# HiLab-git/WSL4MIS

Measured on AMD Instinct MI355X. Metric: training slices/sec (256x256, bs64, unet_cct pCE+GatedCRF), higher is better.
Workload: dtype f32; 1 GPU; unet_cct pce_gatedcrf r=5, 256x256x1 4-class synthetic scribble slices, batch 64/GPU, SGD+poly LR; global_batch=64, parallelism=dp1, crf_radius=5, conv_precision=f32

## Files before the change

### wsl4mis_amd/csrc/wsl_bn.hip

```cpp
#include <stdlib.h>

#include "wsl_rt.h"

namespace wsl {

constexpr int kChunk = 4096;

constexpr int kFinalizeWideFrom = 2048;
static inline int finalize_threads(int nblk) { return nblk >= kFinalizeWideFrom ? 1024 : kThreads; }
template <int NV>
__device__ __forceinline__ void finalize_merge_waves(double (&v)[NV], double* red) {
  const int nw = blockDim.x >> 6, w = threadIdx.x >> 6;
#pragma unroll
  for (int m = 32; m >= 1; m >>= 1)
#pragma unroll
    for (int k = 0; k < NV; ++k) v[k] += __shfl_xor(v[k], m);
  if ((threadIdx.x & 63) == 0)
#pragma unroll
    for (int k = 0; k < NV; ++k) red[k * 16 + w] = v[k];
  __syncthreads();
#pragma unroll
  for (int k = 0; k < NV; ++k) {
    double t[16];
#pragma unroll
// ... 79 lines not shown
      best = v[0];
#pragma unroll
      for (int k = 1; k < 4; ++k)
        if (v[k] > best) best = v[k];
    } else {
#pragma unroll
      for (int k = 0; k < 4; ++k) {
        const int64_t off = (int64_t)(2 * oy + (k >> 1)) * W + 2 * ox + (k & 1);
        const float v = src_value(s, n, c, n * s.bs + c * HW + off, ((int64_t)n * s.C + c) * HW + off);
        if (k == 0 || v > best) best = v;
      }
    }
    out[((int64_t)n * s.C + c) * Ho * Wo + o] = best;
  }
}

__global__ __launch_bounds__(256) void feat_grad_combine_kernel(WslSrc f, const float* ga, int64_t ga_bs,
                                                                const float* gb, int64_t gb_bs, const float* gb_cmask,
                                                                const float* gp, float* g, int H, int W) {
  const int c = blockIdx.y, n = blockIdx.z;
  const int Hc = (H + 1) / 2, Wc = (W + 1) / 2, Ho = H / 2, Wo = W / 2;
  const int64_t HW = (int64_t)H * W;
  const float cm = gb_cmask ? gb_cmask[(int64_t)n * f.C + c] : 1.f;
  const int base = blockIdx.x * kChunk;
  for (int o = base + threadIdx.x; o < base + kChunk && o < Hc * Wc; o += kThreads) {
    const int cy = o / Wc, cx = o - cy * Wc;
    int arg = -1;
    float gpool = 0.f;
    if (gp && cy < Ho && cx < Wo) {
      float best = 0.f;
#pragma unroll
      for (int k = 0; k < 4; ++k) {
        const int64_t off = (int64_t)(2 * cy + (k >> 1)) * W + 2 * cx + (k & 1);
        const float v = src_value(f, n, c, n * f.bs + c * HW + off, ((int64_t)n * f.C + c) * HW + off);
        if (k == 0 || v > best) best = v, arg = k;
      }
      gpool = gp[((int64_t)n * f.C + c) * Ho * Wo + (int64_t)cy * Wo + cx];
    }
#pragma unroll
    for (int k = 0; k < 4; ++k) {
      const int y = 2 * cy + (k >> 1), x = 2 * cx + (k & 1);
      if (y < H && x < W) {
        const int64_t off = (int64_t)y * W + x;
        float v = 0.f;
        if (ga) v = ga[n * ga_bs + c * HW + off];
        if (gb) v = fmaf(gb[n * gb_bs + c * HW + off], cm, v);
        if (k == arg) v += gpool;
        g[((int64_t)n * f.C + c) * HW + off] = v;
      }
    }
  }
}

__global__ __launch_bounds__(256) void feat_grad_combine_bn_kernel(WslSrc f, const float* ga, int64_t ga_bs, const float* gb,
                                                                   int64_t gb_bs, const float* gb_cmask, const float* gp,
                                                                   float* g, int H, int W, const float* bn_mean,
                                                                   const float* bn_invstd, float* bn_part) {
  __shared__ float red[8];
  const int c = blockIdx.y, n = blockIdx.z;
  const int Hc = (H + 1) / 2, Wc = (W + 1) / 2, Ho = H / 2, Wo = W / 2;
  const int64_t HW = (int64_t)H * W;
  const float cm = gb_cmask ? gb_cmask[(int64_t)n * f.C + c] : 1.f;
  const float sc = f.scale[c], sh = f.shift[c], mean = bn_mean[c], invstd = bn_invstd[c];
  const float* fy = f.x + n * f.bs + c * HW;
  float s1 = 0.f, s2 = 0.f;
  const int base = blockIdx.x * kChunk;
  const bool vec = !(H & 1) && !(W & 1) && !(HW & 1) && !(f.bs & 1) && !(ga_bs & 1) && !(gb_bs & 1) &&
                   !(reinterpret_cast<uintptr_t>(f.x) & 7) && !(reinterpret_cast<uintptr_t>(g) & 7) &&
                   !(reinterpret_cast<uintptr_t>(ga) & 7) && !(reinterpret_cast<uintptr_t>(gb) & 7);
  for (int o = base + threadIdx.x; o < base + kChunk && o < Hc * Wc; o += kThreads) {
    const int cy = o / Wc, cx = o - cy * Wc;
    float yv[4], zv[4];
    bool in[4];
    if (vec) {
      const float2 t = *reinterpret_cast<const float2*>(fy + (int64_t)(2 * cy) * W + 2 * cx);
      const float2 b = *reinterpret_cast<const float2*>(fy + (int64_t)(2 * cy + 1) * W + 2 * cx);
      yv[0] = t.x, yv[1] = t.y, yv[2] = b.x, yv[3] = b.y;
#pragma unroll
      for (int k = 0; k < 4; ++k) in[k] = true, zv[k] = fmaf(yv[k], sc, sh);
    } else {
#pragma unroll
      for (int k = 0; k < 4; ++k) {
        const int y = 2 * cy + (k >> 1), x = 2 * cx + (k & 1);
        in[k] = y < H && x < W;
        yv[k] = in[k] ? fy[(int64_t)y * W + x] : 0.f;
        zv[k] = fmaf(yv[k], sc, sh);
      }
    }
    int arg = -1;
    float gpool = 0.f;
    if (gp && cy < Ho && cx < Wo) {
      float best = 0.f;
#pragma unroll
      for (int k = 0; k < 4; ++k) {
        const float v = leaky(zv[k]);
        if (k == 0 || v > best) best = v, arg = k;
      }
      gpool = gp[((int64_t)n * f.C + c) * Ho * Wo + (int64_t)cy * Wo + cx];
    }
    float av[4] = {0.f, 0.f, 0.f, 0.f}, bv[4] = {0.f, 0.f, 0.f, 0.f};
    if (vec) {
      const int64_t o0 = c * HW + (int64_t)(2 * cy) * W + 2 * cx;
      if (ga) {
        const float2 t = *reinterpret_cast<const float2*>(ga + n * ga_bs + o0), b = *reinterpret_cast<const float2*>(ga + n * ga_bs + o0 + W);
        av[0] = t.x, av[1] = t.y, av[2] = b.x, av[3] = b.y;
      }
      if (gb) {
        const float2 t = *reinterpret_cast<const float2*>(gb + n * gb_bs + o0), b = *reinterpret_cast<const float2*>(gb + n * gb_bs + o0 + W);
        bv[0] = t.x, bv[1] = t.y, bv[2] = b.x, bv[3] = b.y;
      }
    }
    float vout[4];
#pragma unroll
    for (int k = 0; k < 4; ++k) {
      vout[k] = 0.f;
      if (in[k]) {
        const int64_t off = (int64_t)(2 * cy + (k >> 1)) * W + 2 * cx + (k & 1);
        float v = 0.f;
        if (ga) v = vec ? av[k] : ga[n * ga_bs + c * HW + off];
        if (gb) v = fmaf(vec ? bv[k] : gb[n * gb_bs + c * HW + off], cm, v);
        if (k == arg) v += gpool;
        if (!vec) g[((int64_t)n * f.C + c) * HW + off] = v;
        vout[k] = v;
        const float d = zv[k] > 0.f ? v : WSL_LEAKY_SLOPE * v;
        s1 += d;
        s2 = fmaf(d, (yv[k] - mean) * invstd, s2);
      }
    }
    if (vec) {
      float* go = g + ((int64_t)n * f.C + c) * HW + (int64_t)(2 * cy) * W + 2 * cx;
      *reinterpret_cast<float2*>(go) = make_float2(vout[0], vout[1]);
      *reinterpret_cast<float2*>(go + W) = make_float2(vout[2], vout[3]);
    }
  }
  s1 = block_sum(s1, red);
  s2 = block_sum(s2, red + 4);
  if (threadIdx.x == 0) {
    float* dst = bn_part + (((int64_t)n * gridDim.x + blockIdx.x) * f.C + c) * 2;
    dst[0] = s1;
    dst[1] = s2;
  }
}

struct BnBwdP {
  const float* g;
  int64_t g_bs;
  const float* y;
  const float* mean;
  const float* invstd;
  const float* gamma;
  const float* beta;
  const uint8_t* emask;
  float es;
  int C, HW, chunks;
  int g_is_d = 0;
};

__device__ __forceinline__ float bn_dz(const BnBwdP& p, int n, int c, int i, float sc, float sh, float mean, float invstd,
                                       float* xhat) {
  const int64_t idx = ((int64_t)n * p.C + c) * p.HW + i;
  const float yv = p.y[idx];
  float d = p.g[n * p.g_bs + (int64_t)c * p.HW + i];
  *xhat = (yv - mean) * invstd;
  if (p.g_is_d) return d;
  if (p.emask) d = p.emask[idx] ? d * p.es : 0.f;
  const float z = fmaf(yv, sc, sh);
  return z > 0.f ? d : WSL_LEAKY_SLOPE * d;
}

__global__ __launch_bounds__(256) void bnact_bwd_reduce_kernel(BnBwdP p, float* part) {
  __shared__ float red[8];
  const int c = blockIdx.y, n = blockIdx.z;
  const float mean = p.mean[c], invstd = p.invstd[c];
  const float sc = p.gamma[c] * invstd, sh = fmaf(-mean, sc, p.beta[c]);
  float s1 = 0.f, s2 = 0.f;
  const int base = blockIdx.x * kChunk;
  for (int i = base + threadIdx.x; i < base + kChunk && i < p.HW; i += kThreads) {
    float xh;
    const float d = bn_dz(p, n, c, i, sc, sh, mean, invstd, &xh);
    s1 += d;
    s2 = fmaf(d, xh, s2);
  }
  s1 = block_sum(s1, red);
  s2 = block_sum(s2, red + 4);
  if (threadIdx.x == 0) {
// ... 512 lines not shown
    return WSL_EWORKSPACE;
  }
  BnBwdP p{g, g_bs, y, mean, invstd, gamma, beta, emask, emask_scale, C, H * W, cdiv(H * W, kChunk)};
  p.g_is_d = g_is_d;
  ProfScope ps(PF_BN_BWD, 0.0, (double)N * C * H * W * (12.0 + (emask && !g_is_d ? 1.0 : 0.0)), stream);
  float* coef = static_cast<float*>(ws);
  dim3 grid(p.chunks, C, N);
  auto al16 = [](const void* q) { return (reinterpret_cast<uintptr_t>(q) & 15) == 0; };
  const bool vec = (H * W) % 4 == 0 && (g_bs % 4) == 0 && al16(g) && al16(y) && al16(dy) &&
                   (!emask || (reinterpret_cast<uintptr_t>(emask) & 3) == 0);
  bnact_bwd_finalize_launch(part, nblk, C, channel_major, (double)N * H * W, dgamma, dbeta, coef, stream);
  uint32_t* pmax = dy_amax ? reinterpret_cast<uint32_t*>(coef + 2 * (size_t)C) : nullptr;
  if (vec) WSL_LAUNCH(bnact_bwd_apply4_kernel, grid, dim3(kThreads), 0, stream, p, coef, dy, pmax);
  else WSL_LAUNCH(bnact_bwd_apply_kernel, grid, dim3(kThreads), 0, stream, p, coef, dy, pmax);
  if (dy_amax) WSL_LAUNCH(amax_fold_kernel, dim3(WSL_SP_AMAX_SLOTS), dim3(kThreads), 0, stream, pmax, N * p.chunks * C, dy_amax);
  return check_launch("bnact_bwd_finish");
}

extern "C" int wsl_bnact_bwd_finish_amax(const float* g, int64_t g_bs, const float* y, const float* mean, const float* invstd,
                                         const float* gamma, const float* beta, const uint8_t* emask, float emask_scale, float* dy,
                                         float* dgamma, float* dbeta, int N, int C, int H, int W, const float* part, int nblk,
                                         int channel_major, void* ws, size_t ws_bytes, uint32_t* dy_amax, void* stream) {
  return bnact_bwd_finish_impl(g, g_bs, y, mean, invstd, gamma, beta, emask, emask_scale, dy, dgamma, dbeta, N, C, H, W, part, nblk,
                               channel_major, ws, ws_bytes, dy_amax, 0, stream);
}

extern "C" int wsl_bnact_bwd_finish_d_amax(const float* d, int64_t d_bs, const float* y, const float* mean, const float* invstd,
                                           const float* gamma, const float* beta, float* dy, float* dgamma, float* dbeta, int N, int C,
                                           int H, int W, const float* part, int nblk, int channel_major, void* ws, size_t ws_bytes,
                                           uint32_t* dy_amax, void* stream) {
  return bnact_bwd_finish_impl(d, d_bs, y, mean, invstd, gamma, beta, nullptr, 1.f, dy, dgamma, dbeta, N, C, H, W, part, nblk,
                               channel_major, ws, ws_bytes, dy_amax, 1, stream);
}

extern "C" int wsl_bnact_bwd_finish(const float* g, int64_t g_bs, const float* y, const float* mean, const float* invstd,
                                    const float* gamma, const float* beta, const uint8_t* emask, float emask_scale, float* dy,
                                    float* dgamma, float* dbeta, int N, int C, int H, int W, const float* part, int nblk,
                                    int channel_major, void* ws, size_t ws_bytes, void* stream) {
  return wsl_bnact_bwd_finish_amax(g, g_bs, y, mean, invstd, gamma, beta, emask, emask_scale, dy, dgamma, dbeta, N, C, H, W, part,
                                   nblk, channel_major, ws, ws_bytes, nullptr, stream);
}

extern "C" int wsl_feat_grad_combine_blocks(int N, int H, int W) {
  return N > 0 && H > 0 && W > 0 ? N * cdiv(((H + 1) / 2) * ((W + 1) / 2), kChunk) : 0;
}

extern "C" int wsl_feat_grad_combine_bn(const WslSrc* f, const float* ga, int64_t ga_bs, const float* gb, int64_t gb_bs,
                                        const float* gb_cmask, const float* gp, float* g, int N, int H, int W,
                                        const float* bn_mean, const float* bn_invstd, float* bn_part, void* stream) {
  WSL_REQUIRE(f && f->x && f->scale && f->shift && !f->emask && !f->cmask && g && N > 0 && H > 0 && W > 0 && f->C > 0,
              "feat_grad_combine_bn: the feature must be a plain BatchNorm + LeakyReLU source");
  WSL_REQUIRE(bn_mean && bn_invstd && bn_part, "feat_grad_combine_bn: null BatchNorm argument");
  ProfScope ps(PF_POOL_FANIN, 0.0, (double)N * f->C * H * W * (4.0 * (ga ? 1 : 0) + 4.0 * (gb ? 1 : 0) + (gp ? 1.0 : 0.0) + 8.0), stream);
  WSL_LAUNCH(feat_grad_combine_bn_kernel, dim3(cdiv(((H + 1) / 2) * ((W + 1) / 2), kChunk), f->C, N), dim3(kThreads), 0,
             stream, *f, ga, ga_bs, gb, gb_bs, gb_cmask, gp, g, H, W, bn_mean, bn_invstd, bn_part);
  return check_launch("feat_grad_combine_bn_kernel");
}

extern "C" size_t wsl_bilinear_up2_fwd_amax_ws_bytes(int N, int C, int h, int w) {
  return N > 0 && C > 0 && h > 0 && w > 0 ? sizeof(uint32_t) * (size_t)N * C * cdiv(2 * h, kUpFR) : 0;
}

extern "C" int wsl_bilinear_up2_fwd_amax(const float* u, float* out, int64_t out_bs, int N, int C, int h, int w, void* ws, size_t ws_bytes,
                                         uint32_t* amax_slots, void* stream) {
  WSL_REQUIRE(u && out && N > 0 && C > 0 && h > 0 && w > 0, "bilinear_up2_fwd: bad args");
  WSL_REQUIRE(out_bs >= (int64_t)C * 4 * h * w, "bilinear_up2_fwd: out batch stride too small");
  if (amax_slots && (!ws || ws_bytes < wsl_bilinear_up2_fwd_amax_ws_bytes(N, C, h, w))) {
    set_error("bilinear_up2_fwd_amax: workspace %zu < %zu", ws ? ws_bytes : (size_t)0, wsl_bilinear_up2_fwd_amax_ws_bytes(N, C, h, w));
    return WSL_EWORKSPACE;
  }
  ProfScope ps(PF_BILINEAR, 0.0, 20.0 * (double)N * C * h * w, stream);
  if (up2_fast_ok(out, out_bs, w) && (reinterpret_cast<uintptr_t>(u) & 15) == 0) {
    const dim3 grid(cdiv(2 * h, kUpFR), C, N);
    uint32_t* pmax = amax_slots ? static_cast<uint32_t*>(ws) : nullptr;
    WSL_LAUNCH(bilinear_up2_fwd4_kernel, grid, dim3(kThreads), 0, stream, u, out, out_bs, C, h, w, ilog2(2 * w) - 2, pmax);
    if (amax_slots) WSL_LAUNCH(amax_fold_kernel, dim3(WSL_SP_AMAX_SLOTS), dim3(kThreads), 0, stream, pmax, (int)(grid.x * grid.y * grid.z), amax_slots);
    return check_launch("bilinear_up2_fwd4_kernel");
  }
  if (amax_slots) {
    WSL_REQUIRE(((int64_t)N * C * h * w) % 4 == 0 && (reinterpret_cast<uintptr_t>(u) & 15) == 0, "bilinear_up2_fwd_amax: source not float4-aligned");
    if (hipMemsetAsync(amax_slots, 0, WSL_SP_AMAX_SLOTS * sizeof(uint32_t), (hipStream_t)stream) != hipSuccess) {
      set_error("bilinear_up2_fwd_amax: clearing the slots failed");
      return WSL_EHIP;
    }
    WSL_LAUNCH(amax_tensor_kernel, dim3(256), dim3(kThreads), 0, stream, u, (int64_t)N * C * h * w / 4, amax_slots);
  }
  if (up2_fast_ok(out, out_bs, w)) {
    const int lw = ilog2(2 * w);
    int rows = 8192 / (2 * w);
    if (rows < (kThreads >> lw)) rows = kThreads >> lw;
    WSL_LAUNCH(bilinear_up2_fwdc_kernel, dim3(cdiv(2 * h, rows), C, N), dim3(kThreads), 0, stream, u, out, out_bs, C, h, w,
               lw, rows);
    return check_launch("bilinear_up2_fwdc_kernel");
  }
  WSL_LAUNCH(bilinear_up2_fwd_kernel, dim3(cdiv(4 * h * w, kChunk), C, N), dim3(kThreads), 0, stream, u, out, out_bs, C,
             h, w);
  return check_launch("bilinear_up2_fwd_kernel");
}

extern "C" int wsl_bilinear_up2_fwd(const float* u, float* out, int64_t out_bs, int N, int C, int h, int w, void* stream) {
  return wsl_bilinear_up2_fwd_amax(u, out, out_bs, N, C, h, w, nullptr, 0, nullptr, stream);
}

extern "C" int wsl_bilinear_up2_bwd(const float* dout, int64_t dout_bs, float* du, int N, int C, int h, int w,
                                    void* stream) {
  WSL_REQUIRE(dout && du && N > 0 && C > 0 && h > 0 && w > 0, "bilinear_up2_bwd: bad args");
  WSL_REQUIRE(dout_bs >= (int64_t)C * 4 * h * w, "bilinear_up2_bwd: dout batch stride too small");
  ProfScope ps(PF_BILINEAR, 0.0, 20.0 * (double)N * C * h * w, stream);
// ... 14 lines not shown
```

### wsl4mis_amd/csrc/wsl_conv2.hip

```cpp
#include <stdlib.h>

#include "wsl_rt.h"

namespace wsl {

struct Src2 {
  const float* x;
  const uint8_t* emask;
  const float* scale;
  const float* shift;
  const float* cmask;
  int64_t bs;
  int C;
  float es;
};

struct Conv2P {
  Src2 a, b;
  const float* wp;
  const float* bias;
  float* y;
  int64_t y_bs;
  int N, H, W, Ci, Co, tiles_x, tiles_y;
  float* stat_part;
// ... 398 lines not shown
#define WSL_MARK(k)
#endif
  WSL_MARK(0);
  issue(0);
  for (int c = tid; c < Ci; c += kThreads) {
    const bool ina = c < p.a.C;
    const Src2& s = ina ? p.a : p.b;
    const int ch = ina ? c : c - p.a.C;
    tab[c] = s.scale ? make_float2(s.scale[ch], s.shift[ch]) : make_float2(1.f, 0.f);
    cm_l[c] = s.cmask ? s.cmask[(int64_t)n * s.C + ch] : 1.f;
  }
  if (owner && !pvalid) {
#pragma unroll
    for (int i = 0; i < C::NLD; ++i)
      *reinterpret_cast<float4*>(in_t + i * (C::G * C::PLANE) + loff) = make_float4(0.f, 0.f, 0.f, 0.f);
  }

  v4f acc[C::MT][C::NT];
#pragma unroll
  for (int i = 0; i < C::MT; ++i)
#pragma unroll
    for (int j = 0; j < C::NT; ++j) acc[i][j] = v4f{0.f, 0.f, 0.f, 0.f};
  int abase[C::MT];
#pragma unroll
  for (int i = 0; i < C::MT; ++i) {
    const int mt = wave * C::MT + i;
    abase[i] = (lane >> 4) * C::PLANE + (mt / C::SEGS) * C::ROWP + (mt % C::SEGS) * 16 + (lane & 15) + (C::PADL - C::P);
  }
  const int bbase = (lane >> 4) * C::CSTR + (lane & 15);
  __syncthreads();
  WSL_MARK(1);
  for (int c0 = 0; c0 < Ci; c0 += KC) {
#ifndef WSL_HOST_EMUL
    const int mk = 2 + 6 * (c0 / KC < 4 ? c0 / KC : 3);
    if (tl) __builtin_amdgcn_s_waitcnt(0);
#endif
    WSL_MARK(mk);
    if (!WSL_ABLATED(p, 2) || c0 == 0) commit(c0);
    WSL_MARK(mk + 1);
    __syncthreads();
    WSL_MARK(mk + 2);
    if (c0 + KC < Ci && !WSL_ABLATED(p, 2)) issue(c0 + KC);
    WSL_MARK(mk + 3);
    if (!WSL_ABLATED(p, 1)) conv2_mfma_stages<C, KS, KC, KC / 4>(in_t, w_t, abase, bbase, acc);
    WSL_MARK(mk + 4);
    __syncthreads();
    WSL_MARK(mk + 5);
  }

  if (WSL_ABLATED(p, 4)) {
    if (acc[0][0][0] == 123.456f) p.y[0] = 1.f;
    return;
  }
  float bsum[C::NT];
  {
    constexpr int RPW = C::MT / C::SEGS;
    float* yb = p.y + n * p.y_bs + (int64_t)(co0 + (lane & 15)) * HW + (int64_t)(y0 + wave * RPW) * W + x0 + (lane >> 4) * 4;
#pragma unroll
    for (int j = 0; j < C::NT; ++j) {
      const float bias = p.bias ? p.bias[co0 + j * 16 + (lane & 15)] : 0.f;
      float* yj = yb + (int64_t)j * 16 * HW;
      float bs = 0.f;
#pragma unroll
      for (int i = 0; i < C::MT; ++i) {
        v4f v = acc[i][j];
#pragma unroll
        for (int r = 0; r < 4; ++r) v[r] += bias;
        acc[i][j] = v;
        *reinterpret_cast<float4*>(yj + (i / C::SEGS) * W + (i % C::SEGS) * 16) = make_float4(v[0], v[1], v[2], v[3]);
        bs += (v[0] + v[1]) + (v[2] + v[3]);
      }
      bsum[j] = bs;
    }
  }
#ifndef WSL_HOST_EMUL
  if (tl) {
    __builtin_amdgcn_s_waitcnt(0);
    WSL_MARK(26);
    if (tid == 0) tl[30] = __builtin_amdgcn_s_memrealtime();
    return;
  }
#endif
  if constexpr (C::MT * C::NT * 4 <= 32) if (p.bn.part) {
    constexpr int RPW = C::MT / C::SEGS;
    float s1[C::NT], s2[C::NT];
#pragma unroll
    for (int j = 0; j < C::NT; ++j) {
      const int co = co0 + j * 16 + (lane & 15);
      const float mean = p.bn.st[co], invstd = p.bn.st[Co + co], sc = p.bn.st[2 * Co + co], sh = p.bn.st[3 * Co + co];
      const int64_t base = ((int64_t)n * Co + co) * HW + (int64_t)(y0 + wave * RPW) * W + x0 + (lane >> 4) * 4;
      BnBwdAcc ba;
#pragma unroll
      for (int i = 0; i < C::MT; ++i) {
        bn_bwd_acc4(p.bn, base + (i / C::SEGS) * W + (i % C::SEGS) * 16, acc[i][j][0], acc[i][j][1], acc[i][j][2], acc[i][j][3],
                    mean, invstd, sc, sh, ba);
      }
      bn_bwd_fold(ba, s1[j], s2[j]);
    }
    bn_bwd_store<C::NT, CO_T>(p.bn, s1, s2, in_t, co0, Co, tile_id, nb);
    return;
  }
  if (p.stat_part) {
    float* red1 = in_t;
    float* red2 = in_t + 4 * CO_T;
    constexpr float cnt = (float)(TH * TW);
#pragma unroll
    for (int j = 0; j < C::NT; ++j) {
      float s = bsum[j];
      s += __shfl_xor(s, 16);
      s += __shfl_xor(s, 32);
      if (lane < 16) red1[wave * CO_T + j * 16 + lane] = s;
    }
    __syncthreads();
#pragma unroll
    for (int j = 0; j < C::NT; ++j) {
      const int col = j * 16 + (lane & 15);
      const float mean_b = (red1[col] + red1[CO_T + col] + red1[2 * CO_T + col] + red1[3 * CO_T + col]) / cnt;
      float q = 0.f;
#pragma unroll
      for (int i = 0; i < C::MT; ++i)
#pragma unroll
        for (int r = 0; r < 4; ++r) {
          const float d = acc[i][j][r] - mean_b;
          q = fmaf(d, d, q);
        }
      q += __shfl_xor(q, 16);
      q += __shfl_xor(q, 32);
      if (lane < 16) red2[wave * CO_T + j * 16 + lane] = q;
    }
    __syncthreads();
    if (wave == 0 && lane < 16) {
#pragma unroll
      for (int j = 0; j < C::NT; ++j) {
        const int col = j * 16 + lane, co = co0 + col;
        float* dst = p.stat_part + ((int64_t)co * ((int64_t)nb * p.slots) + (int64_t)tile_id * p.slots) * 2;
        dst[0] = red1[col] + red1[CO_T + col] + red1[2 * CO_T + col] + red1[3 * CO_T + col];
        dst[1] = red2[col] + red2[CO_T + col] + red2[2 * CO_T + col] + red2[3 * CO_T + col];
      }
      if (lane < p.slots && blockIdx.y == 0) p.stat_cnt[tile_id * p.slots + lane] = lane == 0 ? cnt : 0.f;
    }
  }
}
#undef WSL_MARK

template <int KS, int TH, int TW, int CO_T, int KC>
struct Conv2RCfg : Conv2Cfg<KS, TH, TW, CO_T, KC> {
  using B = Conv2Cfg<KS, TH, TW, CO_T, KC>;
  static constexpr size_t SMEM = sizeof(float) * (2 * B::IN_FLOATS + B::W_FLOATS);
// ... 1047 lines not shown
```

### wsl4mis_amd/csrc/wsl_conv4.hip

```cpp
#include <type_traits>

#include "wsl_rt.h"

namespace wsl {

struct WgSmallP {
  const float* a;
  int64_t a_bs;
  const float* a_scale;
  const float* a_shift;
  const float* b;
  int64_t b_bs;
  float* part_dw;
  float* part_db;
  int N, H, W, tiles_x, tiles_y, items, nsplit;
};
struct WgSmallBndP : WgSmallP {
  const float* y = nullptr;
  int64_t y_bs = 0;
  const float* bn_mean = nullptr;
  const float* bn_invstd = nullptr;
  const float* bn_gamma = nullptr;
  const float* bn_coef = nullptr;
};
// ... 379 lines not shown
  if ((H % 8) || (W % 64) || (reinterpret_cast<uintptr_t>(a.x) & 15) || (a.bs & 3)) return false;
  return (reinterpret_cast<uintptr_t>(y) & 15) == 0 && (y_bs & 3) == 0;
}

int conv_cls_launch(const WslSrc& a, const float* wp, const float* bias, float* y, int64_t y_bs, int N, int H, int W,
                    void* stream) {
  ClsP p;
  p.x = a.x, p.x_bs = a.bs, p.scale = a.scale, p.shift = a.shift, p.wp = wp, p.bias = bias, p.y = y, p.y_bs = y_bs;
  p.N = N, p.H = H, p.W = W, p.tiles_x = W / 64, p.tiles_y = H / 8, p.items = N * p.tiles_x * p.tiles_y;
  static bool attr_done = false;
  if (!attr_done) {
    (void)WSL_SET_MAX_DYN_SMEM(conv_cls_kernel, ClsCfg::SMEM);
    attr_done = true;
  }
  int wgs = forced_wgrad_wgs() > 0 ? forced_wgrad_wgs() : 2 * device_cu_count();
  if (wgs > p.items) wgs = p.items;
  const double px = (double)N * H * W;
  void* tok = prof_begin(0, 2.0 * px * 4 * 16 * 9, 4.0 * px * (16 + 4), stream);
  WSL_LAUNCH(conv_cls_kernel, dim3(wgs), dim3(kThreads), ClsCfg::SMEM, stream, p);
  prof_end(tok, stream);
  return check_launch("conv_cls_kernel");
}

struct NkP {
  const float* x;
  int64_t x_bs;
  const float* wp;
  const float* bias;
  float* y;
  int64_t y_bs;
  int N, H, W, tiles_x, tiles_y, items;
  float* stat_part;
  float* stat_cnt;
  int slots;
  BnBwdEpi bn;
};
struct NkApplyP : NkP {
  const float* gamma = nullptr;
  const float* beta = nullptr;
  const float* coef = nullptr;
};

template <int CI, int TH_ = 8, int TW_ = 64>
struct NkCfg {
  static constexpr int TH = TH_, TW = TW_, SEGW = TW / 16;
  static constexpr int PADL = 4, ROWP = TW + 2 * PADL, ROWS = TH + 2, ROWP4 = ROWP / 4, POS = ROWS * ROWP4;
  static constexpr int PLANE = ((ROWS * ROWP - 16 + 31) / 32) * 32 + 16;
  static constexpr int NG = CI == 4 ? 9 : 3;
  static constexpr size_t SMEM = sizeof(float) * (CI * PLANE + 8 * 16);
  static_assert(POS <= 256 && (CI == 1 || CI == 4) && TH * TW == 512, "one float4 position per thread");
};

constexpr int kNk16MinW = 2;
template <int CI, int TH = 8, int TW = 64, bool NHWC = false, int PASS = 0>
__global__ __launch_bounds__(256, kNk16MinW) void conv_nk16_kernel(std::conditional_t<PASS == 2, NkApplyP, NkP> p) {
  using C = NkCfg<CI, TH, TW>;
  WSL_DYN_SMEM(smem);
  float* in_t = reinterpret_cast<float*>(smem);
  float* red = in_t + CI * C::PLANE;
  const int tid = threadIdx.x, lane = tid & 63, wave = tid >> 6;
  const int H = p.H, W = p.W, HW = H * W;
  const int c16 = lane & 15, k4 = lane >> 4;

  float bw[C::NG];
  int aoff[C::NG];
#pragma unroll
  for (int g = 0; g < C::NG; ++g) {
    if (CI == 4) {
      bw[g] = p.wp[(g * 4 + k4) * 16 + c16];
      aoff[g] = k4 * C::PLANE + (g / 3) * C::ROWP + (g % 3);
    } else {
      const int tap = 4 * g + k4;
      bw[g] = tap < 9 ? p.wp[tap * 16 + c16] : 0.f;
      aoff[g] = tap < 9 ? (tap / 3) * C::ROWP + (tap % 3) : 0;
    }
  }
  const float bias = p.bias ? p.bias[c16] : 0.f;

  const int pty = tid / C::ROWP4, ptx4 = tid - pty * C::ROWP4;
  const bool owner = tid < C::POS;
  const int loff = pty * C::ROWP + ptx4 * 4;
  const int it0 = (int)((int64_t)blockIdx.x * p.items / gridDim.x), it1 = (int)((int64_t)(blockIdx.x + 1) * p.items / gridDim.x);
  float4 pre[CI];
  bool pok = false;
  auto tile_of = [&](int item, int& n, int& y0, int& x0) {
    int q = item;
    const int tx = q % p.tiles_x;
    q /= p.tiles_x;
    const int ty = q % p.tiles_y;
    n = q / p.tiles_y, y0 = ty * C::TH, x0 = tx * C::TW;
  };
  auto issue = [&](int item) __attribute__((always_inline)) {
    int n, y0, x0;
    tile_of(item, n, y0, x0);
    const int gy = y0 + pty - 1, gx = x0 + ptx4 * 4 - C::PADL;
    pok = owner && gy >= 0 && gy < H && gx >= 0 && gx < W;
    const uint32_t off = pok ? (uint32_t)(gy * W + gx) : 0u;
    const float* xb = p.x + n * p.x_bs;
#pragma unroll
    for (int i = 0; i < CI; ++i) pre[i] = *reinterpret_cast<const float4*>(xb + (int64_t)i * HW + off);
  };
  auto commit = [&]() __attribute__((always_inline)) {
    if (owner) {
#pragma unroll
      for (int i = 0; i < CI; ++i)
        *reinterpret_cast<float4*>(in_t + i * C::PLANE + loff) = pok ? pre[i] : make_float4(0.f, 0.f, 0.f, 0.f);
    }
  };

  if (it0 < it1) issue(it0);
  for (int item = it0; item < it1; ++item) {
    commit();
    __syncthreads();
    if (item + 1 < it1) issue(item + 1);
    int n, y0, x0;
    tile_of(item, n, y0, x0);
    v4f acc[8];
#pragma unroll
    for (int sg = 0; sg < 8; ++sg) {
      acc[sg] = v4f{bias, bias, bias, bias};
      const float* ab = in_t + ((8 * wave + sg) / C::SEGW) * C::ROWP + (C::PADL - 1) + 16 * ((8 * wave + sg) % C::SEGW) + c16;
#pragma unroll
      for (int g = 0; g < C::NG; ++g) acc[sg] = WSL_MFMA16(ab[aoff[g]], bw[g], acc[sg]);
    }
    if constexpr (PASS == 2) {
      const float mean = p.bn.st[c16], invstd = p.bn.st[16 + c16];
      const float sc = p.gamma[c16] * invstd, sh = fmaf(-mean, sc, p.beta[c16]);
      const float c1 = p.coef[2 * c16], c2 = p.coef[2 * c16 + 1];
      const float* yin = p.bn.y + ((int64_t)n * 16 + c16) * HW + (int64_t)y0 * W + x0 + 4 * k4;
      float* yb = p.y + n * p.y_bs + (int64_t)c16 * HW + (int64_t)y0 * W + x0 + 4 * k4;
#pragma unroll
      for (int sg = 0; sg < 8; ++sg) {
        const int off = ((8 * wave + sg) / C::SEGW) * W + 16 * ((8 * wave + sg) % C::SEGW);
        const float4 yv = *reinterpret_cast<const float4*>(yin + off);
        const float y4[4] = {yv.x, yv.y, yv.z, yv.w};
        float v[4];
#pragma unroll
        for (int k = 0; k < 4; ++k) {
          const float z = fmaf(y4[k], sc, sh);
          const float d = z > 0.f ? acc[sg][k] : WSL_LEAKY_SLOPE * acc[sg][k];
          v[k] = bn_bwd_dy(d, bn_bwd_xhat(y4[k], mean, invstd), sc, c1, c2);
        }
        *reinterpret_cast<float4*>(yb + off) = make_float4(v[0], v[1], v[2], v[3]);
      }
    } else if constexpr (PASS == 1) {
    } else if constexpr (NHWC) {
      float* yb = p.y + n * p.y_bs + ((int64_t)y0 * W + x0 + 4 * k4) * 16 + c16;
#pragma unroll
      for (int sg = 0; sg < 8; ++sg)
#pragma unroll
        for (int r = 0; r < 4; ++r)
          yb[((int64_t)((8 * wave + sg) / C::SEGW) * W + 16 * ((8 * wave + sg) % C::SEGW) + r) * 16] = acc[sg][r];
    } else {
    float* yb = p.y + n * p.y_bs + (int64_t)c16 * HW + (int64_t)y0 * W + x0 + 4 * k4;
#pragma unroll
    for (int sg = 0; sg < 8; ++sg)
      *reinterpret_cast<float4*>(yb + ((8 * wave + sg) / C::SEGW) * W + 16 * ((8 * wave + sg) % C::SEGW)) =
          make_float4(acc[sg][0], acc[sg][1], acc[sg][2], acc[sg][3]);
    }

    if (PASS != 2 && p.bn.part) {
      const float mean = p.bn.st[c16], invstd = p.bn.st[16 + c16], sc = p.bn.st[32 + c16], sh = p.bn.st[48 + c16];
      const int64_t base = ((int64_t)n * 16 + c16) * HW + (int64_t)y0 * W + x0 + 4 * k4;
      BnBwdAcc ba;
#pragma unroll
      for (int sg = 0; sg < 8; ++sg)
        bn_bwd_acc4(p.bn, base + ((8 * wave + sg) / C::SEGW) * W + 16 * ((8 * wave + sg) % C::SEGW), acc[sg][0], acc[sg][1], acc[sg][2], acc[sg][3], mean, invstd, sc,
                    sh, ba);
      float s1[1], s2[1];
      bn_bwd_fold(ba, s1[0], s2[0]);
      bn_bwd_store<1, 16>(p.bn, s1, s2, red, 0, 16, item, p.items);
    } else if (PASS == 0 && p.stat_part) {
      constexpr float cnt = (float)(C::TH * C::TW);
      float* red1 = red;
      float* red2 = red + 64;
      float bs = 0.f;
#pragma unroll
      for (int sg = 0; sg < 8; ++sg) bs += (acc[sg][0] + acc[sg][1]) + (acc[sg][2] + acc[sg][3]);
      bs += __shfl_xor(bs, 16);
      bs += __shfl_xor(bs, 32);
      if (lane < 16) red1[wave * 16 + lane] = bs;
      __syncthreads();
      const float mean_b = (red1[c16] + red1[16 + c16] + red1[32 + c16] + red1[48 + c16]) / cnt;
      float q = 0.f;
#pragma unroll
      for (int sg = 0; sg < 8; ++sg)
#pragma unroll
        for (int e = 0; e < 4; ++e) {
          const float d = acc[sg][e] - mean_b;
          q = fmaf(d, d, q);
        }
      q += __shfl_xor(q, 16);
      q += __shfl_xor(q, 32);
      if (lane < 16) red2[wave * 16 + lane] = q;
      __syncthreads();
      if (wave == 0 && lane < 16) {
        float* dst = p.stat_part + ((int64_t)lane * ((int64_t)p.items * p.slots) + (int64_t)item * p.slots) * 2;
        dst[0] = red1[lane] + red1[16 + lane] + red1[32 + lane] + red1[48 + lane];
        dst[1] = red2[lane] + red2[16 + lane] + red2[32 + lane] + red2[48 + lane];
        if (lane < p.slots) p.stat_cnt[item * p.slots + lane] = lane == 0 ? cnt : 0.f;
      }
    }
    __syncthreads();
  }
}

bool conv_nk16_eligible(const WslSrc& a, const WslSrc* b, const float* y, int64_t y_bs, int H, int W, int Co, int ks, int th, int tw) {
  if (ks != 3 || Co != 16 || (a.C != 1 && a.C != 4) || (b && b->C > 0) || a.scale || a.emask || a.cmask) return false;
  if (th != 8 || tw != 64 || (H % 8) || (W % 64) || (reinterpret_cast<uintptr_t>(a.x) & 15) || (a.bs & 3)) return false;
  return (reinterpret_cast<uintptr_t>(y) & 15) == 0 && (y_bs & 3) == 0 && (int64_t)16 * H * W < (int64_t(1) << 31);
}

template <int CI, int TH, int TW>
static int launch_nk16(NkP& p, bool dgrad, void* stream) {
  using C = NkCfg<CI, TH, TW>;
  auto kern = conv_nk16_kernel<CI, TH, TW>;
  p.tiles_x = p.W / TW, p.tiles_y = p.H / TH;
  static bool attr_done = false;
  if (!attr_done) {
    (void)WSL_SET_MAX_DYN_SMEM(kern, C::SMEM);
    attr_done = true;
  }
  int wgs = kNk16MinW * device_cu_count();
  if (wgs > p.items) wgs = p.items;
  const double px = (double)p.N * p.H * p.W;
  void* tok = prof_begin(dgrad ? PF_CONV_DGRAD : PF_CONV_FWD, 2.0 * px * CI * 16 * 9, 4.0 * px * (16 + CI) + bn_epi_bytes(p.bn, px * 16), stream);
  WSL_LAUNCH(kern, dim3(wgs), dim3(kThreads), C::SMEM, stream, p);
  prof_end(tok, stream);
  return check_launch("conv_nk16_kernel");
}

int conv_nk16_launch(const WslSrc& a, const float* wp, const float* bias, float* y, int64_t y_bs, int N, int H, int W, bool dgrad,
                     float* stat_part, float* stat_cnt, int slots, const BnBwdEpi* bn, int* bn_done, void* stream) {
  NkP p;
  p.x = a.x, p.x_bs = a.bs, p.wp = wp, p.bias = bias, p.y = y, p.y_bs = y_bs;
  p.N = N, p.H = H, p.W = W, p.tiles_x = W / 64, p.tiles_y = H / 8, p.items = N * p.tiles_x * p.tiles_y;
  p.stat_part = stat_part, p.stat_cnt = stat_cnt, p.slots = slots;
  const bool bn_ok = bn && bn->part;
  if (bn_ok) p.bn = *bn;
  if (bn_done) *bn_done = bn_ok ? 1 : 0;
#ifdef WSL_EXPERIMENTS
  static const int nhwc = WSL_TUNE("WSL_NK16_NHWC", 0);
  if (nhwc) {
    auto kern = a.C == 4 ? conv_nk16_kernel<4, 8, 64, true> : conv_nk16_kernel<1, 8, 64, true>;
    p.tiles_x = W / 64, p.tiles_y = H / 8;
    int wgs = kNk16MinW * device_cu_count();
    if (wgs > p.items) wgs = p.items;
    WSL_LAUNCH(kern, dim3(wgs), dim3(kThreads), (a.C == 4 ? NkCfg<4>::SMEM : NkCfg<1>::SMEM), stream, p);
    return check_launch("conv_nk16_kernel(nhwc probe)");
  }
  static const int wide = WSL_TUNE("WSL_NK16_WIDE", 0);
  if (wide && W % 128 == 0) return a.C == 4 ? launch_nk16<4, 4, 128>(p, dgrad, stream) : launch_nk16<1, 4, 128>(p, dgrad, stream);
#endif
  return a.C == 4 ? launch_nk16<4, 8, 64>(p, dgrad, stream) : launch_nk16<1, 8, 64>(p, dgrad, stream);
}

template <int PASS>
static int launch_nk16_pass(std::conditional_t<PASS == 2, NkApplyP, NkP>& p, void* stream) {
  using C = NkCfg<4, 8, 64>;
  auto kern = conv_nk16_kernel<4, 8, 64, false, PASS>;
  static bool attr_done = false;
  if (!attr_done) {
    (void)WSL_SET_MAX_DYN_SMEM(kern, C::SMEM);
    attr_done = true;
  }
  int wgs = kNk16MinW * device_cu_count();
  if (wgs > p.items) wgs = p.items;
  const double px = (double)p.N * p.H * p.W, flops = 2.0 * px * 4 * 16 * 9;
  void* tok = PASS == 1 ? prof_begin(PF_CONV_DGRAD, flops, 4.0 * px * (4 + 16), stream)
                        : prof_begin(PF_CONV_DGRAD, 0.0, 4.0 * px * (4 + 16 + 16), stream, flops);
  WSL_LAUNCH(kern, dim3(wgs), dim3(kThreads), C::SMEM, stream, p);
  prof_end(tok, stream);
  return check_launch(PASS == 1 ? "conv_nk16_kernel(statistics pass)" : "conv_nk16_kernel(apply pass)");
}

static void nk16_fill(NkP& p, const WslSrc& a, const float* wp, int N, int H, int W, const BnBwdEpi& bn) {
  p.x = a.x, p.x_bs = a.bs, p.wp = wp, p.bias = nullptr, p.y = nullptr, p.y_bs = (int64_t)16 * H * W;
  p.N = N, p.H = H, p.W = W, p.tiles_x = W / 64, p.tiles_y = H / 8, p.items = N * p.tiles_x * p.tiles_y;
  p.stat_part = nullptr, p.stat_cnt = nullptr, p.slots = 1;
  p.bn = bn;
}

int conv_nk16_stats_launch(const WslSrc& a, const float* wp, int N, int H, int W, const BnBwdEpi& bn, void* stream) {
  NkP p;
  nk16_fill(p, a, wp, N, H, W, bn);
  return launch_nk16_pass<1>(p, stream);
}

int conv_nk16_apply_launch(const WslSrc& a, const float* wp, int N, int H, int W, const BnBwdEpi& bn, const float* gamma,
                           const float* beta, const float* coef, float* dy, void* stream) {
  NkApplyP p;
  nk16_fill(p, a, wp, N, H, W, bn);
  p.y = dy, p.gamma = gamma, p.beta = beta, p.coef = coef;
  return launch_nk16_pass<2>(p, stream);
}

#ifdef WSL_EXPERIMENTS
#ifndef WSL_HOST_EMUL
template <int SHAPE>
__global__ __launch_bounds__(256) void mfma_stream_kernel(float* out, int iters) {
  typedef float v4 __attribute__((ext_vector_type(4)));
  typedef float v16 __attribute__((ext_vector_type(16)));
  const float a = 1.0f + threadIdx.x * 1e-6f, b = 0.5f;
  float r = 0.f;
  if (SHAPE == 1) {
    v16 acc[4];
    for (int i = 0; i < 4; ++i) for (int k = 0; k < 16; ++k) acc[i][k] = 0.f;
    for (int it = 0; it < iters; ++it) {
#pragma unroll
      for (int u = 0; u < 4; ++u)
#pragma unroll
        for (int i = 0; i < 4; ++i) acc[i] = __builtin_amdgcn_mfma_f32_32x32x2f32(a, b, acc[i], 0, 0, 0);
    }
    for (int i = 0; i < 4; ++i) r += acc[i][0];
  } else {
    v4 acc[16];
    for (int i = 0; i < 16; ++i) acc[i] = v4{0.f, 0.f, 0.f, 0.f};
    for (int it = 0; it < iters; ++it) {
#pragma unroll
// ... 176 lines not shown
```

Baseline: 4163 slices/s.

## Specialize fan-in kernel by operand presence and prefetch BN epilogue inputs

The feature-gradient fan-in kernel is now templated on vectorization and on which gradient inputs are present, so dead branches and per-element runtime checks disappear. Two conv kernels (conv2 1x1 tile and nk16) load the BatchNorm epilogue's y and mask values before the MFMA loop, so the global loads overlap with compute. The nk16 loop also reorders commit and sync around the next tile's issue, and raises occupancy and grid size for the stats and apply passes. These add register pressure and a more complex synchronization order in exchange for hiding memory latency.

Result: no change. 4188 slices/s (median of 6 runs) (+0.6%).

```diff
diff --git a/wsl4mis_amd/csrc/wsl_bn.hip b/wsl4mis_amd/csrc/wsl_bn.hip
--- a/wsl4mis_amd/csrc/wsl_bn.hip
+++ b/wsl4mis_amd/csrc/wsl_bn.hip
@@ -155,6 +155,7 @@
   }
 }
 
+template <bool VEC, bool GA, bool GB, bool GP>
 __global__ __launch_bounds__(256) void feat_grad_combine_bn_kernel(WslSrc f, const float* ga, int64_t ga_bs, const float* gb,
                                                                    int64_t gb_bs, const float* gb_cmask, const float* gp,
                                                                    float* g, int H, int W, const float* bn_mean,
@@ -168,27 +169,58 @@
   const float* fy = f.x + n * f.bs + c * HW;
   float s1 = 0.f, s2 = 0.f;
   const int base = blockIdx.x * kChunk;
-  const bool vec = !(H & 1) && !(W & 1) && !(HW & 1) && !(f.bs & 1) && !(ga_bs & 1) && !(gb_bs & 1) &&
-                   !(reinterpret_cast<uintptr_t>(f.x) & 7) && !(reinterpret_cast<uintptr_t>(g) & 7) &&
-                   !(reinterpret_cast<uintptr_t>(ga) & 7) && !(reinterpret_cast<uintptr_t>(gb) & 7);
-  for (int o = base + threadIdx.x; o < base + kChunk && o < Hc * Wc; o += kThreads) {
+  if constexpr (VEC) {
+    const float* gap = GA ? ga + n * ga_bs + c * HW : nullptr;
+    const float* gbp = GB ? gb + n * gb_bs + c * HW : nullptr;
+    const float* gpp = GP ? gp + ((int64_t)n * f.C + c) * Ho * Wo : nullptr;
+    float* gop = g + ((int64_t)n * f.C + c) * HW;
+    for (int o = base + threadIdx.x; o < base + kChunk && o < Hc * Wc; o += kThreads) {
+      const int cy = o / Wc, cx = o - cy * Wc;
+      const int64_t r0 = (int64_t)(2 * cy) * W + 2 * cx;
+      const float2 yt = *reinterpret_cast<const float2*>(fy + r0), yb = *reinterpret_cast<const float2*>(fy + r0 + W);
+      float2 at = make_float2(0.f, 0.f), ab = at, bt = at, bb = at;
+      float gpool = 0.f;
+      if constexpr (GA) at = *reinterpret_cast<const float2*>(gap + r0), ab = *reinterpret_cast<const float2*>(gap + r0 + W);
+      if constexpr (GB) bt = *reinterpret_cast<const float2*>(gbp + r0), bb = *reinterpret_cast<const float2*>(gbp + r0 + W);
+      if constexpr (GP) gpool = gpp[(int64_t)cy * Wo + cx];
+      const float yv[4] = {yt.x, yt.y, yb.x, yb.y}, av[4] = {at.x, at.y, ab.x, ab.y}, bv[4] = {bt.x, bt.y, bb.x, bb.y};
+      float zv[4];
+#pragma unroll
+      for (int k = 0; k < 4; ++k) zv[k] = fmaf(yv[k], sc, sh);
+      int arg = -1;
+      if constexpr (GP) {
+        float best = 0.f;
+#pragma unroll
+        for (int k = 0; k < 4; ++k) {
+          const float v = leaky(zv[k]);
+          if (k == 0 || v > best) best = v, arg = k;
+        }
+      }
+      float vout[4];
+#pragma unroll
+      for (int k = 0; k < 4; ++k) {
+        float v = 0.f;
+        if constexpr (GA) v = av[k];
+        if constexpr (GB) v = fmaf(bv[k], cm, v);
+        if (k == arg) v += gpool;
+        vout[k] = v;
+        const float d = zv[k] > 0.f ? v : WSL_LEAKY_SLOPE * v;
+        s1 += d;
+        s2 = fmaf(d, (yv[k] - mean) * invstd, s2);
+      }
+      *reinterpret_cast<float2*>(gop + r0) = make_float2(vout[0], vout[1]);
+      *reinterpret_cast<float2*>(gop + r0 + W) = make_float2(vout[2], vout[3]);
+    }
+  } else for (int o = base + threadIdx.x; o < base + kChunk && o < Hc * Wc; o += kThreads) {
     const int cy = o / Wc, cx = o - cy * Wc;
     float yv[4], zv[4];
     bool in[4];
-    if (vec) {
-      const float2 t = *reinterpret_cast<const float2*>(fy + (int64_t)(2 * cy) * W + 2 * cx);
-      const float2 b = *reinterpret_cast<const float2*>(fy + (int64_t)(2 * cy + 1) * W + 2 * cx);
-      yv[0] = t.x, yv[1] = t.y, yv[2] = b.x, yv[3] = b.y;
-#pragma unroll
-      for (int k = 0; k < 4; ++k) in[k] = true, zv[k] = fmaf(yv[k], sc, sh);
-    } else {
-#pragma unroll
-      for (int k = 0; k < 4; ++k) {
-        const int y = 2 * cy + (k >> 1), x = 2 * cx + (k & 1);
-        in[k] = y < H && x < W;
-        yv[k] = in[k] ? fy[(int64_t)y * W + x] : 0.f;
-        zv[k] = fmaf(yv[k], sc, sh);
-      }
+#pragma unroll
+    for (int k = 0; k < 4; ++k) {
+      const int y = 2 * cy + (k >> 1), x = 2 * cx + (k & 1);
+      in[k] = y < H && x < W;
+      yv[k] = in[k] ? fy[(int64_t)y * W + x] : 0.f;
+      zv[k] = fmaf(yv[k], sc, sh);
     }
     int arg = -1;
     float gpool = 0.f;
@@ -201,39 +233,19 @@
       }
       gpool = gp[((int64_t)n * f.C + c) * Ho * Wo + (int64_t)cy * Wo + cx];
     }
-    float av[4] = {0.f, 0.f, 0.f, 0.f}, bv[4] = {0.f, 0.f, 0.f, 0.f};
-    if (vec) {
-      const int64_t o0 = c * HW + (int64_t)(2 * cy) * W + 2 * cx;
-      if (ga) {
-        const float2 t = *reinterpret_cast<const float2*>(ga + n * ga_bs + o0), b = *reinterpret_cast<const float2*>(ga + n * ga_bs + o0 + W);
-        av[0] = t.x, av[1] = t.y, av[2] = b.x, av[3] = b.y;
-      }
-      if (gb) {
-        const float2 t = *reinterpret_cast<const float2*>(gb + n * gb_bs + o0), b = *reinterpret_cast<const float2*>(gb + n * gb_bs + o0 + W);
-        bv[0] = t.x, bv[1] = t.y, bv[2] = b.x, bv[3] = b.y;
-      }
-    }
-    float vout[4];
 #pragma unroll
     for (int k = 0; k < 4; ++k) {
-      vout[k] = 0.f;
       if (in[k]) {
         const int64_t off = (int64_t)(2 * cy + (k >> 1)) * W + 2 * cx + (k & 1);
         float v = 0.f;
-        if (ga) v = vec ? av[k] : ga[n * ga_bs + c * HW + off];
-        if (gb) v = fmaf(vec ? bv[k] : gb[n * gb_bs + c * HW + off], cm, v);
+        if (ga) v = ga[n * ga_bs + c * HW + off];
+        if (gb) v = fmaf(gb[n * gb_bs + c * HW + off], cm, v);
         if (k == arg) v += gpool;
-        if (!vec) g[((int64_t)n * f.C + c) * HW + off] = v;
-        vout[k] = v;
+        g[((int64_t)n * f.C + c) * HW + off] = v;
         const float d = zv[k] > 0.f ? v : WSL_LEAKY_SLOPE * v;
         s1 += d;
         s2 = fmaf(d, (yv[k] - mean) * invstd, s2);
       }
-    }
-    if (vec) {
-      float* go = g + ((int64_t)n * f.C + c) * HW + (int64_t)(2 * cy) * W + 2 * cx;
-      *reinterpret_cast<float2*>(go) = make_float2(vout[0], vout[1]);
-      *reinterpret_cast<float2*>(go + W) = make_float2(vout[2], vout[3]);
     }
   }
   s1 = block_sum(s1, red);
@@ -852,8 +864,26 @@
               "feat_grad_combine_bn: the feature must be a plain BatchNorm + LeakyReLU source");
   WSL_REQUIRE(bn_mean && bn_invstd && bn_part, "feat_grad_combine_bn: null BatchNorm argument");
   ProfScope ps(PF_POOL_FANIN, 0.0, (double)N * f->C * H * W * (4.0 * (ga ? 1 : 0) + 4.0 * (gb ? 1 : 0) + (gp ? 1.0 : 0.0) + 8.0), stream);
-  WSL_LAUNCH(feat_grad_combine_bn_kernel, dim3(cdiv(((H + 1) / 2) * ((W + 1) / 2), kChunk), f->C, N), dim3(kThreads), 0,
-             stream, *f, ga, ga_bs, gb, gb_bs, gb_cmask, gp, g, H, W, bn_mean, bn_invstd, bn_part);
+  const int64_t HW = (int64_t)H * W;
+  const bool vec = !(H & 1) && !(W & 1) && !(HW & 1) && !(f->bs & 1) && !(ga_bs & 1) && !(gb_bs & 1) &&
+                   !(reinterpret_cast<uintptr_t>(f->x) & 7) && !(reinterpret_cast<uintptr_t>(g) & 7) &&
+                   !(reinterpret_cast<uintptr_t>(ga) & 7) && !(reinterpret_cast<uintptr_t>(gb) & 7);
+  const dim3 grid(cdiv(((H + 1) / 2) * ((W + 1) / 2), kChunk), f->C, N);
+#define WSL_FANIN(VEC_, GA_, GB_, GP_)                                                                                        \
+  WSL_LAUNCH((feat_grad_combine_bn_kernel<VEC_, GA_, GB_, GP_>), grid, dim3(kThreads), 0, stream, *f, ga, ga_bs, gb, gb_bs, \
+             gb_cmask, gp, g, H, W, bn_mean, bn_invstd, bn_part)
+  switch (vec ? (ga ? 4 : 0) | (gb ? 2 : 0) | (gp ? 1 : 0) : -1) {
+    case 0: WSL_FANIN(true, false, false, false); break;
+    case 1: WSL_FANIN(true, false, false, true); break;
+    case 2: WSL_FANIN(true, false, true, false); break;
+    case 3: WSL_FANIN(true, false, true, true); break;
+    case 4: WSL_FANIN(true, true, false, false); break;
+    case 5: WSL_FANIN(true, true, false, true); break;
+    case 6: WSL_FANIN(true, true, true, false); break;
+    case 7: WSL_FANIN(true, true, true, true); break;
+    default: WSL_FANIN(false, false, false, false); break;
+  }
+#undef WSL_FANIN
   return check_launch("feat_grad_combine_bn_kernel");
 }
 
diff --git a/wsl4mis_amd/csrc/wsl_conv2.hip b/wsl4mis_amd/csrc/wsl_conv2.hip
--- a/wsl4mis_amd/csrc/wsl_conv2.hip
+++ b/wsl4mis_amd/csrc/wsl_conv2.hip
@@ -474,6 +474,35 @@
     if (acc[0][0][0] == 123.456f) p.y[0] = 1.f;
     return;
   }
+  constexpr bool BN_EPI = C::MT * C::NT * 4 <= 32;
+  constexpr bool BN_PRE = BN_EPI && KS == 1 && TH == 8 && TW == 32 && CO_T == 32;
+  constexpr int NPRE = BN_PRE ? C::MT * C::NT : 1;
+  float4 ypre[NPRE];
+  uint32_t mpre[NPRE];
+  float stpre[C::NT][4];
+  if constexpr (BN_PRE) if (p.bn.part) {
+    constexpr int RPW = C::MT / C::SEGS;
+    const int64_t base = ((int64_t)n * Co + co0 + (lane & 15)) * HW + (int64_t)(y0 + wave * RPW) * W + x0 + (lane >> 4) * 4;
+#pragma unroll
+    for (int j = 0; j < C::NT; ++j)
+#pragma unroll
+      for (int i = 0; i < C::MT; ++i)
+        ypre[j * C::MT + i] = *reinterpret_cast<const float4*>(p.bn.y + base + (int64_t)j * 16 * HW + (i / C::SEGS) * W + (i % C::SEGS) * 16);
+#pragma unroll
+    for (int j = 0; j < C::NT; ++j)
+#pragma unroll
+      for (int k = 0; k < 4; ++k) stpre[j][k] = p.bn.st[k * Co + co0 + j * 16 + (lane & 15)];
+    if (p.bn.emask) {
+#pragma unroll
+      for (int j = 0; j < C::NT; ++j)
+#pragma unroll
+        for (int i = 0; i < C::MT; ++i)
+          mpre[j * C::MT + i] = *reinterpret_cast<const uint32_t*>(p.bn.emask + base + (int64_t)j * 16 * HW + (i / C::SEGS) * W + (i % C::SEGS) * 16);
+    } else {
+#pragma unroll
+      for (int q = 0; q < NPRE; ++q) mpre[q] = 0u;
+    }
+  }
   float bsum[C::NT];
   {
     constexpr int RPW = C::MT / C::SEGS;
@@ -503,19 +532,28 @@
     return;
   }
 #endif
-  if constexpr (C::MT * C::NT * 4 <= 32) if (p.bn.part) {
+  if constexpr (BN_EPI) if (p.bn.part) {
     constexpr int RPW = C::MT / C::SEGS;
     float s1[C::NT], s2[C::NT];
 #pragma unroll
     for (int j = 0; j < C::NT; ++j) {
-      const int co = co0 + j * 16 + (lane & 15);
-      const float mean = p.bn.st[co], invstd = p.bn.st[Co + co], sc = p.bn.st[2 * Co + co], sh = p.bn.st[3 * Co + co];
-      const int64_t base = ((int64_t)n * Co + co) * HW + (int64_t)(y0 + wave * RPW) * W + x0 + (lane >> 4) * 4;
       BnBwdAcc ba;
-#pragma unroll
-      for (int i = 0; i < C::MT; ++i) {
-        bn_bwd_acc4(p.bn, base + (i / C::SEGS) * W + (i % C::SEGS) * 16, acc[i][j][0], acc[i][j][1], acc[i][j][2], acc[i][j][3],
-                    mean, invstd, sc, sh, ba);
+      if constexpr (BN_PRE) {
+        const float mean = stpre[j][0], invstd = stpre[j][1], sc = stpre[j][2], sh = stpre[j][3];
+#pragma unroll
+        for (int i = 0; i < C::MT; ++i) {
+          bn_bwd_acc4v(p.bn, ypre[j * C::MT + i], mpre[j * C::MT + i], acc[i][j][0], acc[i][j][1], acc[i][j][2], acc[i][j][3], mean, invstd,
+                       sc, sh, ba);
+        }
+      } else {
+        const int co = co0 + j * 16 + (lane & 15);
+        const float mean = p.bn.st[co], invstd = p.bn.st[Co + co], sc = p.bn.st[2 * Co + co], sh = p.bn.st[3 * Co + co];
+        const int64_t base = ((int64_t)n * Co + co) * HW + (int64_t)(y0 + wave * RPW) * W + x0 + (lane >> 4) * 4;
+#pragma unroll
+        for (int i = 0; i < C::MT; ++i) {
+          bn_bwd_acc4(p.bn, base + (i / C::SEGS) * W + (i % C::SEGS) * 16, acc[i][j][0], acc[i][j][1], acc[i][j][2], acc[i][j][3],
+                      mean, invstd, sc, sh, ba);
+        }
       }
       bn_bwd_fold(ba, s1[j], s2[j]);
     }
diff --git a/wsl4mis_amd/csrc/wsl_conv4.hip b/wsl4mis_amd/csrc/wsl_conv4.hip
--- a/wsl4mis_amd/csrc/wsl_conv4.hip
+++ b/wsl4mis_amd/csrc/wsl_conv4.hip
@@ -455,8 +455,9 @@
 };
 
 constexpr int kNk16MinW = 2;
+constexpr int kNk16PassWgs = 3;
 template <int CI, int TH = 8, int TW = 64, bool NHWC = false, int PASS = 0>
-__global__ __launch_bounds__(256, kNk16MinW) void conv_nk16_kernel(std::conditional_t<PASS == 2, NkApplyP, NkP> p) {
+__global__ __launch_bounds__(256, (PASS ? kNk16PassWgs : kNk16MinW)) void conv_nk16_kernel(std::conditional_t<PASS == 2, NkApplyP, NkP> p) {
   using C = NkCfg<CI, TH, TW>;
   WSL_DYN_SMEM(smem);
   float* in_t = reinterpret_cast<float*>(smem);
@@ -511,13 +512,42 @@
     }
   };
 
-  if (it0 < it1) issue(it0);
+  const bool bn_y = PASS != 0 || p.bn.part != nullptr, bn_m = PASS != 2 && bn_y && p.bn.emask != nullptr;
+  float e_mean = 0.f, e_invstd = 0.f, e_sc = 0.f, e_sh = 0.f, e_c1 = 0.f, e_c2 = 0.f;
+  if constexpr (PASS == 2) {
+    e_mean = p.bn.st[c16], e_invstd = p.bn.st[16 + c16];
+    e_sc = p.gamma[c16] * e_invstd, e_sh = fmaf(-e_mean, e_sc, p.beta[c16]);
+    e_c1 = p.coef[2 * c16], e_c2 = p.coef[2 * c16 + 1];
+  } else if (bn_y) {
+    e_mean = p.bn.st[c16], e_invstd = p.bn.st[16 + c16], e_sc = p.bn.st[32 + c16], e_sh = p.bn.st[48 + c16];
+  }
+
+  if (it0 < it1) {
+    issue(it0);
+    commit();
+  }
   for (int item = it0; item < it1; ++item) {
-    commit();
     __syncthreads();
-    if (item + 1 < it1) issue(item + 1);
     int n, y0, x0;
     tile_of(item, n, y0, x0);
+    const int64_t ebase = ((int64_t)n * 16 + c16) * HW + (int64_t)y0 * W + x0 + 4 * k4;
+    float4 ypre[8];
+    uint32_t mpre[8];
+    if (bn_y) {
+#pragma unroll
+      for (int sg = 0; sg < 8; ++sg)
+        ypre[sg] = *reinterpret_cast<const float4*>(p.bn.y + ebase + ((8 * wave + sg) / C::SEGW) * W + 16 * ((8 * wave + sg) % C::SEGW));
+    }
+    if (bn_m) {
+#pragma unroll
+      for (int sg = 0; sg < 8; ++sg)
+        mpre[sg] = *reinterpret_cast<const uint32_t*>(p.bn.emask + ebase + ((8 * wave + sg) / C::SEGW) * W + 16 * ((8 * wave + sg) % C::SEGW));
+    } else {
+#pragma unroll
+      for (int sg = 0; sg < 8; ++sg) mpre[sg] = 0u;
+    }
+    issue(item + 1 < it1 ? item + 1 : item);
+    WSL_SCHED_BARRIER();
     v4f acc[8];
 #pragma unroll
     for (int sg = 0; sg < 8; ++sg) {
@@ -526,17 +556,15 @@
 #pragma unroll
       for (int g = 0; g < C::NG; ++g) acc[sg] = WSL_MFMA16(ab[aoff[g]], bw[g], acc[sg]);
     }
+    __syncthreads();
+    commit();
     if constexpr (PASS == 2) {
-      const float mean = p.bn.st[c16], invstd = p.bn.st[16 + c16];
-      const float sc = p.gamma[c16] * invstd, sh = fmaf(-mean, sc, p.beta[c16]);
-      const float c1 = p.coef[2 * c16], c2 = p.coef[2 * c16 + 1];
-      const float* yin = p.bn.y + ((int64_t)n * 16 + c16) * HW + (int64_t)y0 * W + x0 + 4 * k4;
+      const float mean = e_mean, invstd = e_invstd, sc = e_sc, sh = e_sh, c1 = e_c1, c2 = e_c2;
       float* yb = p.y + n * p.y_bs + (int64_t)c16 * HW + (int64_t)y0 * W + x0 + 4 * k4;
+      float4 dyq[8];
 #pragma unroll
       for (int sg = 0; sg < 8; ++sg) {
-        const int off = ((8 * wave + sg) / C::SEGW) * W + 16 * ((8 * wave + sg) % C::SEGW);
-        const float4 yv = *reinterpret_cast<const float4*>(yin + off);
-        const float y4[4] = {yv.x, yv.y, yv.z, yv.w};
+        const float y4[4] = {ypre[sg].x, ypre[sg].y, ypre[sg].z, ypre[sg].w};
         float v[4];
 #pragma unroll
         for (int k = 0; k < 4; ++k) {
@@ -544,8 +572,11 @@
           const float d = z > 0.f ? acc[sg][k] : WSL_LEAKY_SLOPE * acc[sg][k];
           v[k] = bn_bwd_dy(d, bn_bwd_xhat(y4[k], mean, invstd), sc, c1, c2);
         }
-        *reinterpret_cast<float4*>(yb + off) = make_float4(v[0], v[1], v[2], v[3]);
+        dyq[sg] = make_float4(v[0], v[1], v[2], v[3]);
       }
+#pragma unroll
+      for (int sg = 0; sg < 8; ++sg)
+        *reinterpret_cast<float4*>(yb + ((8 * wave + sg) / C::SEGW) * W + 16 * ((8 * wave + sg) % C::SEGW)) = dyq[sg];
     } else if constexpr (PASS == 1) {
     } else if constexpr (NHWC) {
       float* yb = p.y + n * p.y_bs + ((int64_t)y0 * W + x0 + 4 * k4) * 16 + c16;
@@ -562,14 +593,12 @@
           make_float4(acc[sg][0], acc[sg][1], acc[sg][2], acc[sg][3]);
     }
 
-    if (PASS != 2 && p.bn.part) {
-      const float mean = p.bn.st[c16], invstd = p.bn.st[16 + c16], sc = p.bn.st[32 + c16], sh = p.bn.st[48 + c16];
-      const int64_t base = ((int64_t)n * 16 + c16) * HW + (int64_t)y0 * W + x0 + 4 * k4;
+    if (PASS == 1 || (PASS == 0 && p.bn.part)) {
+      const float mean = e_mean, invstd = e_invstd, sc = e_sc, sh = e_sh;
       BnBwdAcc ba;
 #pragma unroll
       for (int sg = 0; sg < 8; ++sg)
-        bn_bwd_acc4(p.bn, base + ((8 * wave + sg) / C::SEGW) * W + 16 * ((8 * wave + sg) % C::SEGW), acc[sg][0], acc[sg][1], acc[sg][2], acc[sg][3], mean, invstd, sc,
-                    sh, ba);
+        bn_bwd_acc4v(p.bn, ypre[sg], mpre[sg], acc[sg][0], acc[sg][1], acc[sg][2], acc[sg][3], mean, invstd, sc, sh, ba);
       float s1[1], s2[1];
       bn_bwd_fold(ba, s1[0], s2[0]);
       bn_bwd_store<1, 16>(p.bn, s1, s2, red, 0, 16, item, p.items);
@@ -604,7 +633,6 @@
         if (lane < p.slots) p.stat_cnt[item * p.slots + lane] = lane == 0 ? cnt : 0.f;
       }
     }
-    __syncthreads();
   }
 }
 
@@ -624,7 +652,7 @@
     (void)WSL_SET_MAX_DYN_SMEM(kern, C::SMEM);
     attr_done = true;
   }
-  int wgs = kNk16MinW * device_cu_count();
+  int wgs = forced_wgrad_wgs() > 0 ? forced_wgrad_wgs() : kNk16MinW * device_cu_count();
   if (wgs > p.items) wgs = p.items;
   const double px = (double)p.N * p.H * p.W;
   void* tok = prof_begin(dgrad ? PF_CONV_DGRAD : PF_CONV_FWD, 2.0 * px * CI * 16 * 9, 4.0 * px * (16 + CI) + bn_epi_bytes(p.bn, px * 16), stream);
@@ -667,7 +695,7 @@
     (void)WSL_SET_MAX_DYN_SMEM(kern, C::SMEM);
     attr_done = true;
   }
-  int wgs = kNk16MinW * device_cu_count();
+  int wgs = forced_wgrad_wgs() > 0 ? forced_wgrad_wgs() : kNk16PassWgs * device_cu_count();
   if (wgs > p.items) wgs = p.items;
   const double px = (double)p.N * p.H * p.W, flops = 2.0 * px * 4 * 16 * 9;
   void* tok = PASS == 1 ? prof_begin(PF_CONV_DGRAD, flops, 4.0 * px * (4 + 16), stream)
```
